# AnastasiaBelenkii/tendermint

Measured on AMD Instinct MI355X. Metric: ed25519 verifies/sec at 1/2/4/8 GPUs + p50 VerifyCommit latency, 150 vals, higher is better.
Workload: dtype int32

## Files before the change

__graft_entry__.py:

```python
import os
import subprocess
import sys

REPO = os.path.dirname(os.path.abspath(__file__))


def build() -> None:
    env = dict(os.environ, PYTORCH_ROCM_ARCH="gfx950")
    subprocess.run(["make", "-s", "-C", os.path.join(REPO, "tendermint_amd", "csrc")], check=True, env=env)
    subprocess.run(["bash", os.path.join(REPO, "tools", "build_checks.sh")], check=True, env=env)
    subprocess.run(["make", "-s", "-C", os.path.join(REPO, "oracle")], check=True)
    subprocess.run(["make", "-s", "-C", os.path.join(REPO, "tendermint_amd", "testing", "csrc")], check=True)
    subprocess.run(["make", "-s", "-C", os.path.join(REPO, "tests", "native")], check=True)
    subprocess.run(["make", "-s", "-C", os.path.join(REPO, "tests", "native", "secp")], check=True)
    subprocess.run(["make", "-s", "-C", os.path.join(REPO, "tests", "native", "secpcomb")], check=True)
    subprocess.run(["make", "-s", "-C", os.path.join(REPO, "tests", "native", "merkle")], check=True)
    subprocess.run(["make", "-s", "-C", os.path.join(REPO, "tests", "native", "pcache")], check=True)
    subprocess.run(["make", "-s", "-C", os.path.join(REPO, "tests", "native", "colorder")], check=True)
    subprocess.run(["make", "-s", "-C", os.path.join(REPO, "tests", "native", "split")], check=True)
    subprocess.run(["make", "-s", "-C", os.path.join(REPO, "tests", "native", "blocks")], check=True)
    subprocess.run(["make", "-s", "-C", os.path.join(REPO, "tests", "native", "voteext")], check=True)
    subprocess.run(["make", "-s", "-C", os.path.join(REPO, "tests", "native", "proofops")], check=True)
    subprocess.run(["make", "-s", "-C", os.path.join(REPO, "tests", "native", "stage")], check=True)
    subprocess.run(["make", "-s", "-C", os.path.join(REPO, "tests", "native", "results")], check=True)
    subprocess.run(["make", "-s", "-C", os.path.join(REPO, "tests", "native", "keyorder")], check=True)
    subprocess.run(["make", "-s", "-C", os.path.join(REPO, "tests", "native", "blockwire")], check=True)
    sys.path.insert(0, REPO)
    import tendermint_amd
    from tendermint_amd import _native
    _native.lib()


def smoke() -> None:
    sys.path.insert(0, REPO)
    sys.path.insert(0, os.path.join(REPO, "oracle"))
    import numpy as np
    import torch
    from tendermint_amd import _native
    from tendermint_amd.testing.factory import make_c2_batch
    import oracle_c

    assert torch.cuda.is_available(), "smoke() needs a GPU"
    ctx = _native.Context(1)
    b = make_c2_batch(1000, seed=7)
    ok_g, vec_g = ctx.ed25519_verify_batch(b.pk, b.sig, b.msg, b.off)
    ok_o, vec_o = oracle_c.ed25519_verify_packed(b.pk, b.sig, b.msg, b.off, threads=4)
    assert ok_g == ok_o and np.array_equal(vec_g, vec_o), "GPU validity vector differs from the oracle"
    info = _native.build_info()
    print(f"smoke ok: {int(vec_g.sum())}/{b.n} valid, bit-exact vs oracle; {info['version']} "
          f"(src digest of this tree {'matches' if info['src_match'] else 'DIFFERS: ' + info['src_digest_tree']})")


if __name__ == "__main__":
    build()
    smoke()
```

tendermint_amd/csrc/msm.h:

```cpp
#pragma once
#include <stddef.h>
#include <stdint.h>
#include "curve25519.h"
#include "split.h"

namespace tmv {

constexpr uint32_t kMsmWideRows = 65536;
constexpr int kMsmChunkMax = 32;
constexpr uint32_t kMsmEmpty = 0xffffffffu;
constexpr uint32_t kMsmCompactGroups = 2048;
constexpr uint32_t kMsmSplitGroups = 4096;
constexpr uint32_t kMsmSplitMax = 8;
constexpr int kMsmSortBlock = 256;
constexpr uint32_t kSubGroupLog2 = 3;
constexpr uint32_t kSubGroup = 1u << kSubGroupLog2;

struct alignas(16) niels_pt {
  fe ypx, ymx, xy2d;
  int32_t pad[2];
};

#ifndef TMV_NIELS_PAIR
#define TMV_NIELS_PAIR 0
#endif
constexpr uint32_t kNielsPer = TMV_NIELS_PAIR ? 2 : 1;

TMV_HD niels_pt niels_negate(const niels_pt &p) {
  niels_pt r;
  r.ypx = p.ymx;
  r.ymx = p.ypx;
  fe_neg(r.xy2d, p.xy2d);
  r.pad[0] = r.pad[1] = 0;
  return r;
}

TMV_HD void niels_store(niels_pt *pts, uint64_t i, const niels_pt &p) {
  if (kNielsPer == 2) {
    pts[2 * i] = p;
    pts[2 * i + 1] = niels_negate(p);
  } else {
    pts[i] = p;
  }
}

struct MsmParams {
  uint32_t m_log2;
  uint32_t c;
  uint32_t W;
  uint32_t WR;
  uint32_t H;
  uint32_t cap;
  uint32_t groups;
  uint32_t P;
  uint32_t L;
  uint32_t merged;
  uint32_t sub;
  uint32_t Ws;
  uint32_t Wa;
  uint32_t Wl;
  uint32_t split_max;
  uint32_t split;

  TMV_HD uint32_t m() const { return 1u << m_log2; }
  TMV_HD uint32_t WL() const { return (129 + m_log2 + c - 1) / c; }
  TMV_HD uint32_t buckets_per_group() const { return W * H; }
  TMV_HD uint32_t bucket(uint32_t w, uint32_t i) const { return w * H + i; }
  TMV_HD uint32_t chunks_per_group() const { return cap / L; }
  TMV_HD uint32_t wpart_slots() const { return P; }

  static MsmParams make(uint32_t n, uint32_t m_log2, uint32_t c, bool merged = false) {
    MsmParams p;
    p.m_log2 = m_log2;
    p.c = c;
    p.merged = merged ? 1 : 0;
    p.sub = 0;
    p.WR = (129 + c - 1) / c;
    p.W = merged ? p.WR : (254 + c - 1) / c;
    p.H = 1u << (c - 1);
    const uint32_t m = 1u << m_log2;
    const uint32_t rw = p.WR > p.WL() ? p.WR : p.WL();
    const uint32_t slots = merged ? m * p.WR : m * rw + (m + 1) * p.W;
    p.cap = (slots + kMsmChunkMax - 1) / kMsmChunkMax * kMsmChunkMax;
    const uint32_t mean = (merged ? m : 2 * m) / p.H;
    p.L = mean <= 16 ? 16 : 32;
    p.groups = (n + m - 1) >> m_log2;
    uint32_t best = ~0u;
    for (uint32_t P = 1; P <= p.H; P *= 2) {
      uint32_t lg = 0;
      while ((p.H / P) >> (lg + 1)) lg++;
      const uint32_t chain = 2 * (p.H / P) + 3 * P + lg;
      if (chain < best) { best = chain; p.P = P; }
    }
    if ((uint64_t)p.groups * p.W >= kMsmWideRows) p.P = 1;
    p.Ws = split_windows(p.W);
    p.Wa = p.Ws > p.WR ? p.Ws : p.WR;
    p.Wl = p.Ws > p.WL() ? p.Ws : p.WL();
    p.split_max = 0;
    p.split = 0;
    return p;
  }
};

struct MsmWork {
  niels_pt *pts;
  uint32_t *ent_pt;
  uint32_t *ent_bk;
  uint32_t *bk_start;
  uint32_t *bk_cnt;
  ge_p3 *bk_sum;
  ge_p3 *part_first;
  ge_p3 *part_last;
  uint32_t *join_b;
  uint32_t *join_count;
  ge_p3 *wpart;
  ge_p3 *wsum;
  uint32_t *grp_chunks;
  uint32_t *chunk_end;
  uint32_t compact;
  uint8_t *group_ok;
  uint8_t *sort_ovf;
  uint32_t n_pts;
  uint32_t *fail_count;
  uint32_t *fail_list;
  uint8_t *sub_ok;
  fe *tabR;
  fe *fail_T;
  uint32_t *loc_count;
  uint32_t *fb_count;
  uint32_t *loc_found;
  uint32_t *fb_list;
  const uint8_t *merge_pk;
  uint8_t *grp_split;
  uint32_t *hi_of;
  uint32_t *hi_list;
  uint32_t *uns_list;
  uint32_t *split_cnt;
  uint32_t g_base;
  unsigned long long *ent_total;
  uint32_t *wscal;
  uint32_t *bscal;
  fe *item_pt;

  static size_t max_items(uint32_t n, const MsmParams &p) { return (size_t)n + 2ull * p.groups; }

  static size_t point_slots(uint32_t n, const MsmParams &p) {
    return 2ull * n + 1 + (p.split ? 1 + (size_t)p.groups * p.split_max : 0);
  }
  static size_t bytes(uint32_t n, const MsmParams &p) {
    const size_t G = p.groups, bk = (size_t)G * p.buckets_per_group(), ent = (size_t)G * p.cap;
    const size_t chunks = ent / p.L;
    size_t b = point_slots(n, p) * kNielsPer * sizeof(niels_pt) + 8 * ent + 8 * bk + bk * sizeof(ge_p3) +
// ... 160 lines not shown
```

tendermint_amd/csrc/msm_kernels.hip:

```cpp
#include <hip/hip_runtime.h>
#include <cstdlib>
#include <cstring>
#include "ed25519_core.h"
#include "kernel_util.h"
#include "comb.h"
#include "quad.h"
#include "ktimer.h"
#include "verify_kernels.h"
#include "halfscalar.h"
#include "knobs.h"

#include <algorithm>
#include <atomic>
#include <mutex>
#include <vector>

namespace tmv {

namespace ktimer {
namespace {
struct Pair {
  int k;
  hipEvent_t a, b;
};
std::atomic<bool> g_on{false};
std::mutex g_mu;
std::vector<Pair *> g_done[kCount];
std::vector<hipEvent_t> g_free;
hipEvent_t take_event() {
  hipEvent_t e = nullptr;
  {
    std::lock_guard<std::mutex> lk(g_mu);
    if (!g_free.empty()) { e = g_free.back(); g_free.pop_back(); }
  }
  if (!e && hipEventCreate(&e) != hipSuccess) e = nullptr;
  return e;
}
}

void set(bool on) { g_on.store(on); }
bool on() { return g_on.load(std::memory_order_relaxed); }

void *begin(Kernel k, hipStream_t s) {
  if (!on()) return nullptr;
  Pair *p = new Pair{k, take_event(), take_event()};
  if (!p->a || !p->b || hipEventRecord(p->a, s) != hipSuccess) {
    std::lock_guard<std::mutex> lk(g_mu);
    if (p->a) g_free.push_back(p->a);
    if (p->b) g_free.push_back(p->b);
    delete p;
    return nullptr;
  }
  return p;
}

void end(void *token, hipStream_t s) {
  if (!token) return;
  Pair *p = static_cast<Pair *>(token);
  (void)hipEventRecord(p->b, s);
  std::lock_guard<std::mutex> lk(g_mu);
  g_done[p->k].push_back(p);
}

int read(Kernel k, double *ms, uint64_t *launches) {
  std::vector<Pair *> v;
  {
    std::lock_guard<std::mutex> lk(g_mu);
    v.swap(g_done[k]);
  }
  int rc = 0;
  for (Pair *p : v) {
    float t = 0.f;
    hipError_t e = hipEventSynchronize(p->b);
    if (e == hipSuccess) e = hipEventElapsedTime(&t, p->a, p->b);
    if (e == hipSuccess) {
      *ms += t;
      *launches += 1;
    } else if (!rc) {
      rc = (int)e;
    }
    std::lock_guard<std::mutex> lk(g_mu);
    g_free.push_back(p->a);
    g_free.push_back(p->b);
    delete p;
  }
  return rc;
}

}

namespace {

template <int V>
struct StaticIndex {
  static constexpr int value = V;
};

template <int NW>
struct DigitReader {
  uint32_t wd[NW];
  uint64_t buf;
  uint32_t avail;
  int carry;
  __device__ __forceinline__ void init(const uint32_t *s) {
#pragma unroll
    for (int k = 0; k < NW; k++) wd[k] = s[k];
    buf = 0;
    avail = 0;
    carry = 0;
  }
  __device__ __forceinline__ int next(uint32_t c, bool top) {
    if (avail < c) {
      buf |= (uint64_t)wd[0] << avail;
#pragma unroll
      for (int k = 0; k + 1 < NW; k++) wd[k] = wd[k + 1];
      wd[NW - 1] = 0;
      avail += 32;
    }
    int d = (int)(buf & ((1u << c) - 1)) + carry;
    buf >>= c;
    avail -= c;
    if (!top && d >= (1 << (c - 1))) {
      d -= 1 << c;
      carry = 1;
    } else {
      carry = 0;
    }
    return d;
  }
};

template <int NW, typename F>
__device__ __forceinline__ void for_each_digit(const uint32_t *s, uint32_t windows, const MsmParams &p, F f) {
  DigitReader<NW> rd;
  rd.init(s);
  for (uint32_t w = 0; w < windows; w++) {
    const int d = rd.next(p.c, w + 1 == windows);
    if (d != 0) f(p.bucket(w, (uint32_t)((d < 0 ? -d : d) - 1)), d < 0);
  }
}

__device__ __forceinline__ void p3_add(ge_p3 &a, const ge_p3 &b) {
  ge_cached c;
  ge_p3_to_cached(c, b);
  ge_p1p1 r;
  ge_add(r, a, c);
  ge_p1p1_to_p3(a, r);
}

TMV_HD uint32_t merge_runs(const MsmParams &p) { return p.m() / 2 < 256u ? p.m() / 2 : 256u; }

constexpr uint32_t kSplitWords = 40;
TMV_HD uint32_t sort_words(const MsmParams &p, uint32_t bs) {
  const uint32_t sort = bs * 9 + bs + 1 + 2 * (2 * p.m() + 1);
  const uint32_t merge = 6 * p.m() + 1 + 16 * merge_runs(p);
  return p.W * p.H + (sort > merge ? sort : merge);
}

__device__ __forceinline__ void p3_dbl(ge_p3 &a) {
  ge_p1p1 r;
  ge_p3_dbl(r, a);
  ge_p1p1_to_p3(a, r);
}

}

template <bool SR, bool KM, int BS = kMsmSortBlock, bool LOC = false, bool SPLIT = false>
__global__ void __launch_bounds__(BS)
k_msm_sort(const uint8_t *__restrict__ sig, const uint32_t *__restrict__ idx, const uint32_t *count_ptr, uint32_t n,
           Ed25519Work w, MsmWork mw, MsmParams p, MsmSeed seed, const fe *__restrict__ btab_q, int aligned,
           const uint32_t *__restrict__ key_slot, const uint8_t *__restrict__ key_ok, uint8_t *__restrict__ out,
           uint32_t e_base) {
  extern __shared__ uint32_t smem[];
  const uint32_t cnt = entry_count(count_ptr, n);
  const uint32_t tid = threadIdx.x;
  uint32_t g = blockIdx.x;
  if (g == 0 && tid == 0) *mw.join_count = 0;
  if (LOC) {
    const uint32_t nf = *mw.fail_count;
    if (g == 0 && tid == 0) {
      *mw.loc_count = nf << p.m_log2;
      *mw.fb_count = 0;
      *mw.loc_found = 0;
    }
    if (g >= nf) return;
  }
  const uint32_t slot = g;
  if (LOC) g = mw.fail_list[slot];
  const uint32_t e0 = g << p.m_log2;
  if (!KM && !LOC && g == 0 && tid == 0) {
    niels_pt bp;
    bp.ymx = btab_q[0];
    bp.ypx = btab_q[1];
    bp.xy2d = btab_q[2];
    bp.pad[0] = bp.pad[1] = 0;
    niels_store(mw.pts, mw.n_pts, bp);
    if constexpr (SPLIT) {
      const fe *bh = btab_q + 4 * (2 * kBaseQuadEntries + (p.c - 4));
      bp.ymx = bh[0];
      bp.ypx = bh[1];
      bp.xy2d = bh[2];
      niels_store(mw.pts, mw.n_pts + 1, bp);
    }
    if (mw.fail_count) *mw.fail_count = 0;
  }
  if (e0 >= cnt) return;
  const uint32_t mlive = min(p.m(), cnt - e0);
  const uint32_t WH = p.W * p.H;
  uint32_t *hist = smem;
  uint32_t *red = smem + WH;
  uint32_t *scan = red + BS * 9;

  constexpr int R = 4;
  constexpr int ZW = LOC ? 5 : 4;
  const uint32_t WRz = LOC ? p.WL() : p.WR;
  uint32_t z[R][ZW], wv[R][8];
  bool live[R];
  uint32_t acc[9];
#pragma unroll
  for (int t = 0; t < 9; t++) acc[t] = 0;
  auto weigh = [&](auto rc) {
// ... 165 lines not shown
        if (diff) continue;
        follower[r] = true;
        trun[myslot[r]] = kWant;
      }
      __syncthreads();
#pragma unroll
      for (int r = 0; r < R; r++) {
        if (!leader[r] || trun[myslot[r]] != kWant) continue;
        const uint32_t sl = atomicAdd(nruns, 1u);
        trun[myslot[r]] = sl < RUNS ? sl : kNone;
      }
      __syncthreads();
#pragma unroll
      for (int r = 0; r < R; r++) {
        if (!follower[r]) continue;
        const uint32_t sl = trun[myslot[r]];
        if (sl >= RUNS) continue;
#pragma unroll
        for (int t = 0; t < 8; t++) {
          atomicAdd(&racc[sl * 16 + 2 * t], wv[r][t] & 0xffffu);
          atomicAdd(&racc[sl * 16 + 2 * t + 1], wv[r][t] >> 16);
          wv[r][t] = 0;
        }
      }
      __syncthreads();
#pragma unroll
      for (int r = 0; r < R; r++) {
        if (!leader[r]) continue;
        const uint32_t sl = trun[myslot[r]];
        if (sl >= RUNS) continue;
        uint32_t x[16];
        uint64_t c = 0;
#pragma unroll
        for (int t = 0; t < 8; t++) {
          c += (uint64_t)racc[sl * 16 + 2 * t] + (wv[r][t] & 0xffffu);
          const uint32_t lo16 = (uint32_t)c & 0xffffu;
          c >>= 16;
          c += (uint64_t)racc[sl * 16 + 2 * t + 1] + (wv[r][t] >> 16);
          x[t] = lo16 | (((uint32_t)c & 0xffffu) << 16);
          c >>= 16;
        }
        x[8] = (uint32_t)c;
#pragma unroll
        for (int t = 9; t < 16; t++) x[t] = 0;
        sc_reduce512(wv[r], x);
      }
    }
  }

  bool split_g = false;
  uint32_t hi_pt[R];
  int carry_hi[R], carry_bhi = 0;
  uint32_t *lmask = smem + sort_words(p, BS), *lbad = lmask + 32, *lbase = lmask + 33;
  if constexpr (SPLIT) {
    bool lead[R];
#pragma unroll
    for (int r = 0; r < R; r++) {
      hi_pt[r] = 0;
      carry_hi[r] = 0;
      uint32_t nz = 0;
#pragma unroll
      for (int t = 0; t < 8; t++) nz |= wv[r][t];
      lead[r] = live[r] && nz != 0;
    }
    if (tid < 34) lmask[tid] = 0;
    __syncthreads();
#pragma unroll
    for (int r = 0; r < R; r++) {
      const uint32_t j = tid + r * BS;
      if (lead[r]) atomicOr(&lmask[j >> 5], 1u << (j & 31));
    }
    __syncthreads();
    uint32_t leaders = 0;
    for (uint32_t k = 0; k < (p.m() + 31) / 32; k++) leaders += __popc(lmask[k]);
    split_g = LOC ? mw.grp_split[g] != 0 : leaders <= p.split_max;
    if (tid == 0) {
      mw.grp_split[(LOC ? p.groups : 0) + slot] = split_g ? 1 : 0;
      if (!split_g) {
        mw.uns_list[atomicAdd(&mw.split_cnt[1], 1u)] = slot;
      } else if (!LOC) {
        *lbase = atomicAdd(&mw.split_cnt[0], leaders);
        if (mw.ent_total) {
          atomicAdd(&mw.ent_total[4], 1ull);
          atomicAdd(&mw.ent_total[5], (unsigned long long)leaders);
        }
      }
    }
    if (split_g) {
      if (!LOC) __syncthreads();
#pragma unroll
      for (int r = 0; r < R; r++) {
        if (!live[r]) continue;
        const uint32_t j = tid + r * BS, e = e0 + j;
        uint32_t gslot = kMsmEmpty;
        if (LOC) {
          if (lead[r]) {
            gslot = mw.hi_of[e];
            if (gslot == kMsmEmpty) atomicOr(lbad, 1u);
          }
        } else {
          if (lead[r]) {
            uint32_t rank = __popc(lmask[j >> 5] & ((1u << (j & 31)) - 1));
            for (uint32_t k = 0; k < (j >> 5); k++) rank += __popc(lmask[k]);
            gslot = (mw.g_base + g) * p.split_max + rank;
            mw.hi_list[2 * (*lbase + rank)] = e;
            mw.hi_list[2 * (*lbase + rank) + 1] = gslot;
          }
          mw.hi_of[e] = gslot;
        }
        hi_pt[r] = mw.n_pts + 2 + gslot;
      }
    }
  }
  auto count_split = [&](const uint32_t *s, int &cy) {
    DigitReader<8> rd;
    rd.init(s);
    for (uint32_t w = 0; w < p.W; w++) {
      if (w == p.Ws) cy = rd.carry;
      const int d = rd.next(p.c, w + 1 == p.W);
      if (d != 0) atomicAdd(&hist[p.bucket(split_slot(w, p.Ws, split_g).window, (uint32_t)((d < 0 ? -d : d) - 1))], 1u);
    }
  };

#pragma unroll
  for (int r = 0; r < R; r++) {
    if (!live[r]) continue;
    for_each_digit<ZW>(z[r], WRz, p, [&](uint32_t bk, bool) { atomicAdd(&hist[bk], 1u); });
    if constexpr (SPLIT) count_split(wv[r], carry_hi[r]);
    else if (!KM) for_each_digit<8>(wv[r], p.W, p, [&](uint32_t bk, bool) { atomicAdd(&hist[bk], 1u); });
  }
  if constexpr (SPLIT) {
    if (tid == 0) count_split(bsc, carry_bhi);
  } else {
    if (!KM && tid == 0) for_each_digit<8>(bsc, p.W, p, [&](uint32_t bk, bool) { atomicAdd(&hist[bk], 1u); });
  }
  __syncthreads();

  const uint32_t seg = (WH + BS - 1) / BS;
  const uint32_t lo = min(WH, tid * seg), hi = min(WH, lo + seg);
  uint32_t local = 0;
  for (uint32_t t = lo; t < hi; t++) local += hist[t];
  scan[tid] = local;
  __syncthreads();
  if (tid == 0) {
    uint32_t run = 0;
    for (int t = 0; t < BS; t++) {
      const uint32_t v = scan[t];
      scan[t] = run;
      run += v;
    }
    scan[BS] = run;
  }
  __syncthreads();
  const uint32_t gbase = slot * p.cap;
  const uint32_t bbase = slot * WH;
  const bool ovf = scan[BS] > p.cap || (SPLIT && *lbad != 0);
  if (tid == 0) mw.sort_ovf[(LOC ? p.groups : 0) + slot] = ovf ? 1 : 0;
  if (tid == 0 && !ovf && mw.ent_total) atomicAdd(mw.ent_total, (unsigned long long)scan[BS]);
  if (tid == 0) mw.grp_chunks[slot] = ovf ? 0u : (scan[BS] + p.L - 1) / p.L;
  if (ovf) {
    for (uint32_t t = tid; t < WH; t += BS) {
      mw.bk_start[bbase + t] = gbase;
      mw.bk_cnt[bbase + t] = 0;
    }
    for (uint32_t t = tid; t < p.cap; t += BS) mw.ent_bk[gbase + t] = kMsmEmpty;
    return;
  }
  {
    uint32_t off = scan[tid];
    for (uint32_t t = lo; t < hi; t++) {
      const uint32_t c = hist[t];
      mw.bk_start[bbase + t] = gbase + off;
      mw.bk_cnt[bbase + t] = c;
      hist[t] = off;
      off += c;
    }
  }
  __syncthreads();

  uint32_t *ent_pt = mw.ent_pt + gbase;
  uint32_t *ent_bk = mw.ent_bk + gbase;
  const uint32_t wcap = 2 * p.m() + 1;
  uint32_t *st_pt = scan + BS + 1, *st_bk = st_pt + wcap;
  DigitReader<ZW> rz[R];
  const uint32_t total = scan[BS];
  if constexpr (SPLIT) {
    DigitReader<5> rlo[R], rblo;
    DigitReader<4> rhi[R], rbhi;
    const uint32_t sh = p.c * p.Ws;
    auto high_half = [&](DigitReader<4> &rd, const uint32_t *s, int cy) {
      uint32_t t[9], h[4];
#pragma unroll
      for (int k = 0; k < 8; k++) t[k] = s[k];
      t[8] = 0;
      for (uint32_t i = 0; i < (sh >> 5); i++) {
#pragma unroll
        for (int k = 0; k < 8; k++) t[k] = t[k + 1];
      }
#pragma unroll
      for (int k = 0; k < 4; k++) h[k] = (uint32_t)((((uint64_t)t[k + 1] << 32) | t[k]) >> (sh & 31));
      rd.init(h);
      rd.carry = cy;
    };
#pragma unroll
    for (int r = 0; r < R; r++) {
      rz[r].init(z[r]);
      rlo[r].init(wv[r]);
      high_half(rhi[r], wv[r], carry_hi[r]);
    }
    rblo.init(bsc);
    high_half(rbhi, bsc, carry_bhi);
    const uint32_t Wg = split_g ? (LOC ? p.Wl : p.Wa) : p.W;
    for (uint32_t w = 0; w < Wg; w++) {
      const uint32_t wbeg = hist[p.bucket(w, 0)];
      const uint32_t wend = w + 1 < p.W ? hist[p.bucket(w + 1, 0)] : total;
      __syncthreads();
      auto put = [&](int d, uint32_t pt) {
        if (d == 0) return;
        const uint32_t bk = p.bucket(w, (uint32_t)((d < 0 ? -d : d) - 1));
        const uint32_t pos = atomicAdd(&hist[bk], 1u) - wbeg;
        st_pt[pos] = (pt << 1) | (d < 0 ? 1u : 0u);
        st_bk[pos] = bbase + bk;
      };
      const uint32_t wh = split_g ? w + p.Ws : w;
      const bool lo_on = w < p.Ws, hi_on = wh >= p.Ws && wh < p.W;
#pragma unroll
      for (int r = 0; r < R; r++) {
        if (!live[r]) continue;
        const uint32_t e = e0 + tid + r * BS;
        if (w < WRz) put(rz[r].next(p.c, w + 1 == WRz), 2 * e);
        if (lo_on) put(rlo[r].next(p.c, false), 2 * e + 1);
        if (hi_on) put(rhi[r].next(p.c, wh + 1 == p.W), split_g ? hi_pt[r] : 2 * e + 1);
      }
      if (tid == 0) {
        if (lo_on) put(rblo.next(p.c, false), mw.n_pts);
        if (hi_on) put(rbhi.next(p.c, wh + 1 == p.W), split_g ? mw.n_pts + 1 : mw.n_pts);
      }
      __syncthreads();
      for (uint32_t i = tid; i < wend - wbeg; i += BS) {
        ent_pt[wbeg + i] = st_pt[i];
        ent_bk[wbeg + i] = st_bk[i];
      }
    }
    const uint32_t pad_end = mw.compact ? min(p.cap, (total + p.L - 1) / p.L * p.L) : p.cap;
    for (uint32_t t = total + tid; t < pad_end; t += BS) ent_bk[t] = kMsmEmpty;
    return;
  }
  DigitReader<8> rw[R], rb;
#pragma unroll
  for (int r = 0; r < R; r++) {
    rz[r].init(z[r]);
    rw[r].init(wv[r]);
  }
  rb.init(bsc);
  for (uint32_t w = 0; w < p.W; w++) {
    const uint32_t wbeg = hist[p.bucket(w, 0)];
    const uint32_t wend = w + 1 < p.W ? hist[p.bucket(w + 1, 0)] : total;
    __syncthreads();
#pragma unroll
    for (int r = 0; r < R; r++) {
      if (!live[r]) continue;
      const uint32_t e = e0 + tid + r * BS;
      if (w < WRz) {
        const int d = rz[r].next(p.c, w + 1 == WRz);
        if (d != 0) {
          const uint32_t bk = p.bucket(w, (uint32_t)((d < 0 ? -d : d) - 1));
          const uint32_t pos = atomicAdd(&hist[bk], 1u) - wbeg;
          st_pt[pos] = ((KM ? e : 2 * e) << 1) | (d < 0 ? 1u : 0u);
          st_bk[pos] = bbase + bk;
        }
      }
      if (!KM) {
        const int d = rw[r].next(p.c, w + 1 == p.W);
        if (d != 0) {
          const uint32_t bk = p.bucket(w, (uint32_t)((d < 0 ? -d : d) - 1));
          const uint32_t pos = atomicAdd(&hist[bk], 1u) - wbeg;
          st_pt[pos] = ((2 * e + 1) << 1) | (d < 0 ? 1u : 0u);
          st_bk[pos] = bbase + bk;
        }
      }
    }
    if (!KM && tid == 0) {
      const int d = rb.next(p.c, w + 1 == p.W);
      if (d != 0) {
        const uint32_t bk = p.bucket(w, (uint32_t)((d < 0 ? -d : d) - 1));
        const uint32_t pos = atomicAdd(&hist[bk], 1u) - wbeg;
        st_pt[pos] = (mw.n_pts << 1) | (d < 0 ? 1u : 0u);
        st_bk[pos] = bbase + bk;
      }
    }
    __syncthreads();
    for (uint32_t i = tid; i < wend - wbeg; i += BS) {
      ent_pt[wbeg + i] = st_pt[i];
      ent_bk[wbeg + i] = st_bk[i];
    }
  }
  const uint32_t pad_end = mw.compact ? min(p.cap, (total + p.L - 1) / p.L * p.L) : p.cap;
  for (uint32_t t = total + tid; t < pad_end; t += BS) ent_bk[t] = kMsmEmpty;
// ... 791 lines not shown

static Ed25519Work work_view(Ed25519Work w, uint64_t e0) {
  w.negA += 4 * e0;
  w.Rc += 4 * e0;
  w.k += 8 * e0;
  w.flags += 4 * e0;
  w.tabA += 64 * e0;
  w.hs_buf += 12 * e0;
  w.miss_list += e0;
  w.miss_count += e0 >> 5;
  return w;
}
static MsmWork msm_view(MsmWork mw, const MsmParams &p, uint32_t n, uint64_t g0) {
  const uint64_t e0 = g0 << p.m_log2, wh = (uint64_t)p.W * p.H;
  mw.pts += 2 * e0 * kNielsPer;
  mw.n_pts = (uint32_t)(2ull * n - 2 * e0);
  mw.ent_pt += g0 * p.cap;
  mw.ent_bk += g0 * p.cap;
  mw.bk_start += g0 * wh;
  mw.bk_cnt += g0 * wh;
  mw.bk_sum += g0 * wh;
  mw.part_first += g0 * p.chunks_per_group();
  mw.part_last += g0 * p.chunks_per_group();
  mw.join_b += g0 * p.chunks_per_group();
  mw.join_count += g0;
  mw.grp_chunks += g0;
  mw.chunk_end += g0;
  mw.wpart += g0 * p.W * 2ull * p.P;
  mw.wsum += g0 * p.W;
  mw.group_ok += g0;
  mw.sort_ovf += g0;
  if (mw.grp_split) {
    mw.grp_split += g0;
    mw.hi_of += e0;
    mw.hi_list += 2 * g0 * p.split_max;
    mw.uns_list += g0;
    mw.split_cnt += 2 * g0;
    mw.g_base = (uint32_t)g0;
  }
  if (mw.sub_ok) mw.sub_ok += (g0 << p.m_log2) / kSubGroup;
  if (mw.tabR) mw.tabR += 32 * e0;
  return mw;
}

template <bool SR, bool LOC>
static hipError_t launch_sort(const uint8_t *sig, const uint32_t *idx, const uint32_t *count_ptr, uint32_t n,
                              uint32_t e_base, const fe *btab_q, Ed25519Work w, MsmWork mw, const MsmParams &p,
                              const MsmSeed &seed, uint8_t *out, int aligned, hipStream_t stream) {
  mw.compact = compact_on(p) ? 1 : 0;
  if constexpr (!SR) {
    if (split_on(mw, p)) {
      hipError_t e = hipMemsetAsync(mw.split_cnt, 0, 2 * sizeof(uint32_t), stream);
      if (e != hipSuccess) return e;
      if (p.m_log2 <= 8)
        hipLaunchKernelGGL((k_msm_sort<false, false, 64, LOC, true>), dim3(p.groups), dim3(64), sort_smem(p, 64, true),
                           stream, sig, idx, count_ptr, n, w, mw, p, seed, btab_q, aligned, nullptr, nullptr, out,
                           e_base);
      else
        hipLaunchKernelGGL((k_msm_sort<false, false, kMsmSortBlock, LOC, true>), dim3(p.groups), dim3(kMsmSortBlock),
                           sort_smem(p, kMsmSortBlock, true), stream, sig, idx, count_ptr, n, w, mw, p, seed, btab_q,
                           aligned, nullptr, nullptr, out, e_base);
      return hipGetLastError();
    }
  }
  if (p.m_log2 <= 8)
    hipLaunchKernelGGL((k_msm_sort<SR, false, 64, LOC>), dim3(p.groups), dim3(64), sort_smem(p, 64), stream, sig, idx,
                       count_ptr, n, w, mw, p, seed, btab_q, aligned, nullptr, nullptr, out, e_base);
  else
    hipLaunchKernelGGL((k_msm_sort<SR, false, kMsmSortBlock, LOC>), dim3(p.groups), dim3(kMsmSortBlock),
                       sort_smem(p, kMsmSortBlock), stream, sig, idx, count_ptr, n, w, mw, p, seed, btab_q, aligned,
                       nullptr, nullptr, out, e_base);
  return hipGetLastError();
}

template <bool SR>
static hipError_t launch_part(const uint8_t *pk, const uint8_t *sig, const uint8_t *msg, const uint32_t *msg_off,
                              const uint32_t *idx, const uint32_t *count_ptr, uint32_t n, uint32_t e_base,
                              const fe *btab_q, const strobe_t *prefix, Ed25519Work w, MsmWork mw,
                              const MsmParams &p, const MsmSeed &seed, uint8_t *out, int aligned,
                              hipStream_t stream) {
  w.niels = mw.pts;
  hipError_t e = launch_prep<SR>(pk, sig, msg, msg_off, idx, count_ptr, n, prefix, w, aligned, stream);
  if (e != hipSuccess) return e;
  if ((e = launch_sort<SR, false>(sig, idx, count_ptr, n, e_base, btab_q, w, mw, p, seed, out, aligned, stream)) !=
      hipSuccess)
    return e;
  if (split_on(mw, p)) {
    const uint64_t hb = ((uint64_t)p.groups * p.split_max + kHiBlock / 4 - 1) / (kHiBlock / 4);
    hipLaunchKernelGGL(k_msm_hi_points, dim3((uint32_t)hb), dim3(kHiBlock), 0, stream, w, mw, p);
    if ((e = hipGetLastError()) != hipSuccess) return e;
  }
  return launch_buckets(count_ptr, n, mw, p, stream);
}

template <bool SR>
static hipError_t launch_tail_stages(const uint8_t *sig, const uint32_t *idx, const uint32_t *count_ptr, uint32_t n,
                                     const fe *btab_q, Ed25519Work w, MsmWork mw, const MsmParams &p,
                                     const MsmSeed &seed, uint8_t *out, int aligned, hipStream_t stream) {
  hipError_t e;
  const bool located = locate_enabled(n, p);
  const bool split = split_on(mw, p);
  const uint8_t *gsplit = split ? mw.grp_split : nullptr;
  const bool helped = !located && w.hs_buf && !split;
  const uint32_t hblocks = (p.groups + 15) / 16;
  if (helped) {
    hipLaunchKernelGGL(k_msm_horner_helped<SR>, dim3(hblocks + (n + 63) / 64), dim3(64), 0, stream, count_ptr, n, mw,
                       p, w, hblocks);
// ... 260 lines not shown
```

tendermint_amd/csrc/tmverify_runtime.cpp:

```cpp
#include <hip/hip_runtime.h>
#include <sys/random.h>

#include <cerrno>

#include <algorithm>
#include <array>
#include <atomic>
#include <chrono>
#include <cstdint>
#include <list>
#include <unordered_map>
#include <cstdlib>
#include <cstdio>
#include <cstring>
#include <functional>
#include <memory>
#include <condition_variable>
#include <mutex>
#include <string>
#include <thread>
#include <vector>

#include "../../include/tmverify.h"
#include "ed25519_core.h"
// ... 359 lines not shown
    if (e == hipErrorNotReady) return 1;
    err = e;
    return 2;
  }, g_timeout_ms);
  if (r == tmh::Poll::kTimeout) {
    d.faulted = true;
    set_error("device wait exceeded TMV_DEVICE_TIMEOUT_MS (" + std::to_string(g_timeout_ms) + " ms)");
    return hipErrorNotReady;
  }
  return err;
}
hipError_t wait_event(Device &d, hipEvent_t ev) {
  read_env();
  hipError_t err = hipSuccess;
  const tmh::Poll r = tmh::poll_until([&] {
    const hipError_t e = hipEventQuery(ev);
    if (e == hipSuccess) return 0;
    if (e == hipErrorNotReady) return 1;
    err = e;
    return 2;
  }, g_timeout_ms);
  if (r == tmh::Poll::kTimeout) {
    d.faulted = true;
    set_error("device wait exceeded TMV_DEVICE_TIMEOUT_MS (" + std::to_string(g_timeout_ms) + " ms)");
    return hipErrorNotReady;
  }
  return err;
}
int wait_rc(hipError_t e) { return e == hipErrorNotReady ? TMV_ERR_TIMEOUT : TMV_ERR_LAUNCH; }
int faulted_rc(Device &d) {
  set_error("device timed out earlier (TMV_ERR_TIMEOUT); open a new context");
  return TMV_ERR_TIMEOUT;
}
int use_device(Device &d, void *stream = nullptr, hipStream_t *s = nullptr) {
  const hipError_t e = hipSetDevice(d.id);
  if (e != hipSuccess) { set_error("hipSetDevice", e); return TMV_ERR_NO_DEVICE; }
  if (!s) return 0;
  *s = stream ? static_cast<hipStream_t>(stream) : context_stream(d);
  if (!*s) { set_error("hipStreamCreate failed"); return TMV_ERR_NO_DEVICE; }
  return 0;
}

constexpr double kRunningSumWeight = 3.0;
static double running_sum_weight() {
  const char *e = tmv::ab_knob("TMV_RS_WEIGHT");
  return e ? atof(e) : kRunningSumWeight;
}
static std::atomic<uint32_t> g_split_groups{tmv::kMsmSplitGroups};
static std::atomic<uint32_t> g_split_max{tmv::kMsmSplitMax};
static uint32_t split_max() {
  const char *e = tmv::ab_knob("TMV_SPLIT_MAX");
  return e ? (uint32_t)strtoul(e, nullptr, 10) : g_split_max.load(std::memory_order_relaxed);
}
tmv::MsmParams msm_params(uint32_t n, uint32_t m_log2, uint32_t c, bool merged = false, bool ed_only = false,
                          int sub = -1) {
  const uint32_t lmin = tmv::locate_min_entries();
  if (m_log2 == 0) m_log2 = merged ? 8 : (ed_only && lmin && n >= lmin ? 7 : 6);
  m_log2 = std::max<uint32_t>(5, std::min<uint32_t>(10, m_log2));
  if (c == 0) {
    const double m = double(1u << m_log2), rsw = running_sum_weight();
    double best = 1e30;
    for (uint32_t cc = 4; cc <= 9; cc++) {
      const double W = (254 + cc - 1) / cc, WR = (129 + cc - 1) / cc, H = double(1u << (cc - 1));
      const double cost = merged ? m * WR + 2.2 * WR * H : m * (W + WR) + rsw * W * H;
      if (cost < best) { best = cost; c = cc; }
    }
  }
  c = std::max<uint32_t>(4, std::min<uint32_t>(9, c));
  tmv::MsmParams p = tmv::MsmParams::make(n, m_log2, c, merged);
  if (g_msm_chunk == 16 || g_msm_chunk == 32) p.L = g_msm_chunk;
  if (g_msm_parts && g_msm_parts <= p.H && !(g_msm_parts & (g_msm_parts - 1))) p.P = g_msm_parts;
  p.sub = merged ? 0 : (sub < 0 ? (tmv::subcheck_enabled(m_log2) ? 1 : 0) : (uint32_t)sub);
  const uint32_t sg = g_split_groups.load(std::memory_order_relaxed);
  const uint32_t smax = tmv::split_max_for(p.m(), split_max());
  if (!merged && ed_only && smax && (sg == 1 || (p.P == 1 && p.groups >= sg)) &&
      2ull * n + 2 + (uint64_t)p.groups * smax < (1ull << 31)) {
    p.split = 1;
    p.split_max = smax;
    p.P = 1;
  }
  return p;
}

struct EngineTimer {
  bool on = tmh::host_timing();
  std::chrono::steady_clock::time_point t = std::chrono::steady_clock::now();
  void mark(const char *what, uint32_t n) {
    if (!on) return;
    const auto now = std::chrono::steady_clock::now();
    fprintf(stderr, "[tmv_engine] %-8s %9.3f ms (n=%u)\n", what,
            std::chrono::duration<double, std::milli>(now - t).count(), n);
    t = now;
  }
};

struct Layout {
  size_t pk, sig, off, msg, total;
  Layout(uint32_t n, size_t msg_bytes) {
    pk = 0;
    sig = align16(pk + 32ull * n);
    off = align16(sig + 64ull * n);
    msg = align16(off + 4ull * (n + 1));
    total = align16(msg + std::max<size_t>(msg_bytes, 1));
  }
};

struct LaunchOpts {
  bool batch_eq = false;
  tmv::MsmParams p{};
  tmv::MsmParams p_ed{};
  tmv::MsmParams p_ed_streamed{};
  tmv::MsmSeed seed[2]{};
  int err = 0;
  bool stats = false;
};

std::atomic<int> g_rand_fault_err{0}, g_rand_fault_count{0};

int draw_weight_key(uint8_t key[32]) {
  size_t got = 0;
  while (got < 32) {
    ssize_t r;
    int fc = g_rand_fault_count.load();
    if (fc != 0) {
      if (fc > 0) g_rand_fault_count.fetch_sub(1);
      errno = g_rand_fault_err.load();
      r = -1;
    } else {
      r = getrandom(key + got, 32 - got, 0);
    }
    if (r > 0) {
// ... 818 lines not shown
  else if (!strcmp(kernel, "k_merkle_aunts")) k = tmv::ktimer::kMerkleAunts;
  else if (!strcmp(kernel, "k_merkle_verify_proofs")) k = tmv::ktimer::kMerkleVerify;
  else if (!strcmp(kernel, "k_merkle_leaves")) k = tmv::ktimer::kMerkleLeaves;
  else if (!strcmp(kernel, "k_commit_leaves")) k = tmv::ktimer::kCommitLeaves;
  else if (!strcmp(kernel, "k_vote_ext_signbytes")) k = tmv::ktimer::kVoteExtSignbytes;
  else if (!strcmp(kernel, "k_merkle_digests_long")) k = tmv::ktimer::kMerkleDigestsLong;
  else if (!strcmp(kernel, "k_merkle_value_ops")) k = tmv::ktimer::kMerkleValueOps;
  else if (!strcmp(kernel, "k_result_leaves")) k = tmv::ktimer::kResultLeaves;
  else if (!strcmp(kernel, "k_span_leaves")) k = tmv::ktimer::kSpanLeaves;
  else { set_error("unknown timed kernel"); return TMV_ERR_ARG; }
  *total_ms = 0;
  *launches = 0;
  const int e = tmv::ktimer::read(k, total_ms, launches);
  if (e) { set_error("hipEventElapsedTime", (hipError_t)e); return TMV_ERR_LAUNCH; }
  return 0;
}

const char *tmv_last_error(void) { return g_last_error.c_str(); }
void tmv_internal_set_error(const char *msg) { g_last_error = msg ? msg : ""; }

void tmv_internal_random_fault(int err, int count) {
  g_rand_fault_err = err;
  g_rand_fault_count = count;
}
int tmv_internal_option(const char *name, int64_t value) {
  if (name && !strcmp(name, "half_scalars")) {
    tmv::set_half_scalar_mode((int)value);
    return 0;
  }
  if (name && !strcmp(name, "point_cache_min")) {
    tmv::set_point_cache_min(value < 0 ? 0u : (uint32_t)value);
    return 0;
  }
  if (name && !strcmp(name, "column_tile")) {
    g_column_tile = value;
    return 0;
  }
  if (name && !strcmp(name, "compact_groups")) {
    tmv::set_compact_groups(value < 0 ? 0u : (uint32_t)value);
    return 0;
  }
  if (name && !strcmp(name, "key_merge")) {
    tmv::set_key_merge(value != 0);
    return 0;
  }
  if (name && !strcmp(name, "split_groups")) {
    g_split_groups = value <= 0 ? tmv::kMsmSplitGroups : (uint32_t)value;
    return 0;
  }
  if (name && !strcmp(name, "split_max")) {
    g_split_max = value <= 0 ? tmv::kMsmSplitMax : (uint32_t)value;
    return 0;
  }
  set_error("unknown internal option");
  return TMV_ERR_ARG;
}
int tmv_internal_checks(uint32_t *out3, int reset) {
  if (!out3) { set_error("null argument"); return TMV_ERR_ARG; }
  if (!tmv::read_checks(out3, reset != 0)) {
    set_error("not a TMV_CHECKS build, or the device read failed");
    return TMV_ERR_ARG;
  }
  return 0;
}
int64_t tmv_internal_mixed_stream_chunk(uint64_t free_bytes) {
  read_env();
  return mixed_stream_chunk((size_t)free_bytes);
}
int tmv_internal_draw_key(uint8_t *out32) {
  if (!out32) { set_error("null argument"); return TMV_ERR_ARG; }
  return draw_weight_key(out32);
}

tmv_ctx *tmv_open(uint32_t device_mask) { return tmv_open_logical(device_mask, 1); }

tmv_ctx *tmv_open_logical(uint32_t device_mask, int logical) {
  release_leaked_pins();
  int count = 0;
  hipError_t e = hipGetDeviceCount(&count);
  if (e != hipSuccess || count <= 0) {
    set_error(e != hipSuccess ? std::string("hipGetDeviceCount: ") + hipGetErrorString(e)
                              : std::string("no HIP device visible"));
    return nullptr;
  }
  logical = std::max(1, std::min(8, logical));
  if (logical > 1)
    fprintf(stderr, "tmverify: TEST AID tmv_open_logical: every GPU opened as %d logical devices\n", logical);
  auto ctx = std::make_unique<tmv_ctx>();
  for (int i = 0; i < count && i < 32; i++) {
    if (device_mask != 0 && !(device_mask & (1u << i))) continue;
    for (int k = 0; k < logical; k++) {
      auto d = std::make_unique<Device>();
      d->id = i;
      if (init_device(*d) != 0) {
        tmv_close(ctx.release());
        return nullptr;
      }
      ctx->devs.push_back(std::move(d));
    }
  }
  if (ctx->devs.empty()) {
    set_error("device_mask selects no visible device");
    return nullptr;
  }
  return ctx.release();
}
// ... 1253 lines not shown
```

Measured before the change: 245.7 million.

## Spread split-scalar leader digit work across thread lanes in MSM sort

In the split path of the MSM sort kernel, each leader scalar's low and high halves (plus the base scalar) become separate tasks, each handled by its own thread. The tasks are staged through a shared-memory table so histogram and scatter run in parallel instead of serially per leader and on thread 0 for the base scalar. This is meant to shorten the serial tail of the sort kernel. In exchange it adds shared-memory staging, a launch-bounds occupancy hint for the split variant, and a cap on split_max tied to the sort block size.

Measured after the change: 245.6 million, median of 4. No clear change (-0.0%).

```diff
diff --git a/__graft_entry__.py b/__graft_entry__.py
--- a/__graft_entry__.py
+++ b/__graft_entry__.py
@@ -18,6 +18,7 @@
     subprocess.run(["make", "-s", "-C", os.path.join(REPO, "tests", "native", "pcache")], check=True)
     subprocess.run(["make", "-s", "-C", os.path.join(REPO, "tests", "native", "colorder")], check=True)
     subprocess.run(["make", "-s", "-C", os.path.join(REPO, "tests", "native", "split")], check=True)
+    subprocess.run(["make", "-s", "-C", os.path.join(REPO, "tests", "native", "splitlanes")], check=True)
     subprocess.run(["make", "-s", "-C", os.path.join(REPO, "tests", "native", "blocks")], check=True)
     subprocess.run(["make", "-s", "-C", os.path.join(REPO, "tests", "native", "voteext")], check=True)
     subprocess.run(["make", "-s", "-C", os.path.join(REPO, "tests", "native", "proofops")], check=True)
diff --git a/tendermint_amd/csrc/msm.h b/tendermint_amd/csrc/msm.h
--- a/tendermint_amd/csrc/msm.h
+++ b/tendermint_amd/csrc/msm.h
@@ -3,6 +3,7 @@
 #include <stdint.h>
 #include "curve25519.h"
 #include "split.h"
+#include "split_lanes.h"
 
 namespace tmv {
 
@@ -13,6 +14,7 @@
 constexpr uint32_t kMsmSplitGroups = 4096;
 constexpr uint32_t kMsmSplitMax = 8;
 constexpr int kMsmSortBlock = 256;
+TMV_HD uint32_t sort_block(uint32_t m_log2) { return m_log2 <= 8 ? 64u : (uint32_t)kMsmSortBlock; }
 constexpr uint32_t kSubGroupLog2 = 3;
 constexpr uint32_t kSubGroup = 1u << kSubGroupLog2;
 
@@ -61,6 +63,7 @@
   uint32_t Wl;
   uint32_t split_max;
   uint32_t split;
+  uint32_t lanes;
 
   TMV_HD uint32_t m() const { return 1u << m_log2; }
   TMV_HD uint32_t WL() const { return (129 + m_log2 + c - 1) / c; }
@@ -98,6 +101,7 @@
     p.Wl = p.Ws > p.WL() ? p.Ws : p.WL();
     p.split_max = 0;
     p.split = 0;
+    p.lanes = 0;
     return p;
   }
 };
diff --git a/tendermint_amd/csrc/msm_kernels.hip b/tendermint_amd/csrc/msm_kernels.hip
--- a/tendermint_amd/csrc/msm_kernels.hip
+++ b/tendermint_amd/csrc/msm_kernels.hip
@@ -9,6 +9,7 @@
 #include "verify_kernels.h"
 #include "halfscalar.h"
 #include "knobs.h"
+#include "split_lanes.h"
 
 #include <algorithm>
 #include <atomic>
@@ -96,40 +97,6 @@
   static constexpr int value = V;
 };
 
-template <int NW>
-struct DigitReader {
-  uint32_t wd[NW];
-  uint64_t buf;
-  uint32_t avail;
-  int carry;
-  __device__ __forceinline__ void init(const uint32_t *s) {
-#pragma unroll
-    for (int k = 0; k < NW; k++) wd[k] = s[k];
-    buf = 0;
-    avail = 0;
-    carry = 0;
-  }
-  __device__ __forceinline__ int next(uint32_t c, bool top) {
-    if (avail < c) {
-      buf |= (uint64_t)wd[0] << avail;
-#pragma unroll
-      for (int k = 0; k + 1 < NW; k++) wd[k] = wd[k + 1];
-      wd[NW - 1] = 0;
-      avail += 32;
-    }
-    int d = (int)(buf & ((1u << c) - 1)) + carry;
-    buf >>= c;
-    avail -= c;
-    if (!top && d >= (1 << (c - 1))) {
-      d -= 1 << c;
-      carry = 1;
-    } else {
-      carry = 0;
-    }
-    return d;
-  }
-};
-
 template <int NW, typename F>
 __device__ __forceinline__ void for_each_digit(const uint32_t *s, uint32_t windows, const MsmParams &p, F f) {
   DigitReader<NW> rd;
@@ -166,7 +133,7 @@
 }
 
 template <bool SR, bool KM, int BS = kMsmSortBlock, bool LOC = false, bool SPLIT = false>
-__global__ void __launch_bounds__(BS)
+__global__ void __launch_bounds__(BS, SPLIT ? 3 : 1)
 k_msm_sort(const uint8_t *__restrict__ sig, const uint32_t *__restrict__ idx, const uint32_t *count_ptr, uint32_t n,
            Ed25519Work w, MsmWork mw, MsmParams p, MsmSeed seed, const fe *__restrict__ btab_q, int aligned,
            const uint32_t *__restrict__ key_slot, const uint8_t *__restrict__ key_ok, uint8_t *__restrict__ out,
@@ -438,6 +405,28 @@
   uint32_t hi_pt[R];
   int carry_hi[R], carry_bhi = 0;
   uint32_t *lmask = smem + sort_words(p, BS), *lbad = lmask + 32, *lbase = lmask + 33;
+  constexpr uint32_t kLaneWords = 10;
+  static_assert((BS / 2) * kLaneWords <= BS * 9, "the task table fits red");
+  bool lanes_g = false;
+  uint32_t ntask = 0;
+  auto task_reader = [&](DigitReader<5> &rd) {
+    const SplitTask task = split_task(tid);
+    const uint32_t *row = red + task.rank * kLaneWords;
+    uint32_t th[5];
+#pragma unroll
+    for (int k = 0; k < 5; k++)
+      th[k] = split_half_word([&](uint32_t q) { return row[q]; }, (uint32_t)k, task.hi, p.c, p.Ws);
+    rd.init(th);
+    if (task.hi) {
+      uint32_t s8[8];
+#pragma unroll
+      for (int t = 0; t < 8; t++) s8[t] = row[t];
+      rd.carry = split_carry_in(s8, p.c, p.Ws);
+    }
+    return row[8 + task.hi];
+  };
+  const bool ttop = (tid & 1) != 0;
+  const uint32_t tnw = ttop ? p.W - p.Ws : p.Ws;
   if constexpr (SPLIT) {
     bool lead[R];
 #pragma unroll
@@ -460,6 +449,7 @@
     uint32_t leaders = 0;
     for (uint32_t k = 0; k < (p.m() + 31) / 32; k++) leaders += __popc(lmask[k]);
     split_g = LOC ? mw.grp_split[g] != 0 : leaders <= p.split_max;
+    lanes_g = split_g && p.lanes && split_task_count(leaders) <= (uint32_t)BS;
     if (tid == 0) {
       mw.grp_split[(LOC ? p.groups : 0) + slot] = split_g ? 1 : 0;
       if (!split_g) {
@@ -478,7 +468,11 @@
       for (int r = 0; r < R; r++) {
         if (!live[r]) continue;
         const uint32_t j = tid + r * BS, e = e0 + j;
-        uint32_t gslot = kMsmEmpty;
+        uint32_t gslot = kMsmEmpty, rank = 0;
+        if (lead[r]) {
+          rank = __popc(lmask[j >> 5] & ((1u << (j & 31)) - 1));
+          for (uint32_t k = 0; k < (j >> 5); k++) rank += __popc(lmask[k]);
+        }
         if (LOC) {
           if (lead[r]) {
             gslot = mw.hi_of[e];
@@ -486,8 +480,6 @@
           }
         } else {
           if (lead[r]) {
-            uint32_t rank = __popc(lmask[j >> 5] & ((1u << (j & 31)) - 1));
-            for (uint32_t k = 0; k < (j >> 5); k++) rank += __popc(lmask[k]);
             gslot = (mw.g_base + g) * p.split_max + rank;
             mw.hi_list[2 * (*lbase + rank)] = e;
             mw.hi_list[2 * (*lbase + rank) + 1] = gslot;
@@ -495,7 +487,25 @@
           mw.hi_of[e] = gslot;
         }
         hi_pt[r] = mw.n_pts + 2 + gslot;
-      }
+        if (lanes_g && lead[r]) {
+          uint32_t *row = red + rank * kLaneWords;
+#pragma unroll
+          for (int t = 0; t < 8; t++) row[t] = wv[r][t];
+          row[8] = 2 * e + 1;
+          row[9] = hi_pt[r];
+        }
+      }
+    }
+    if (lanes_g) {
+      if (tid == 0) {
+        uint32_t *row = red + leaders * kLaneWords;
+#pragma unroll
+        for (int t = 0; t < 8; t++) row[t] = bsc[t];
+        row[8] = mw.n_pts;
+        row[9] = mw.n_pts + 1;
+      }
+      __syncthreads();
+      ntask = split_task_count(leaders);
     }
   }
   auto count_split = [&](const uint32_t *s, int &cy) {
@@ -512,11 +522,23 @@
   for (int r = 0; r < R; r++) {
     if (!live[r]) continue;
     for_each_digit<ZW>(z[r], WRz, p, [&](uint32_t bk, bool) { atomicAdd(&hist[bk], 1u); });
-    if constexpr (SPLIT) count_split(wv[r], carry_hi[r]);
-    else if (!KM) for_each_digit<8>(wv[r], p.W, p, [&](uint32_t bk, bool) { atomicAdd(&hist[bk], 1u); });
+    if constexpr (SPLIT) {
+      if (!lanes_g) count_split(wv[r], carry_hi[r]);
+    } else if (!KM) for_each_digit<8>(wv[r], p.W, p, [&](uint32_t bk, bool) { atomicAdd(&hist[bk], 1u); });
   }
   if constexpr (SPLIT) {
-    if (tid == 0) count_split(bsc, carry_bhi);
+    if (lanes_g) {
+      if (tid < ntask) {
+        DigitReader<5> rd;
+        task_reader(rd);
+        for (uint32_t w = 0; w < tnw; w++) {
+          const int d = rd.next(p.c, ttop && w + 1 == tnw);
+          if (d != 0) atomicAdd(&hist[p.bucket(w, (uint32_t)((d < 0 ? -d : d) - 1))], 1u);
+        }
+      }
+    } else if (tid == 0) {
+      count_split(bsc, carry_bhi);
+    }
   } else {
     if (!KM && tid == 0) for_each_digit<8>(bsc, p.W, p, [&](uint32_t bk, bool) { atomicAdd(&hist[bk], 1u); });
   }
@@ -571,6 +593,45 @@
   DigitReader<ZW> rz[R];
   const uint32_t total = scan[BS];
   if constexpr (SPLIT) {
+    auto scatter_windows = [&](uint32_t Wg, auto body) {
+      for (uint32_t w = 0; w < Wg; w++) {
+        const uint32_t wbeg = hist[p.bucket(w, 0)];
+        const uint32_t wend = w + 1 < p.W ? hist[p.bucket(w + 1, 0)] : total;
+        __syncthreads();
+        auto put = [&](int d, uint32_t pt) {
+          if (d == 0) return;
+          const uint32_t bk = p.bucket(w, (uint32_t)((d < 0 ? -d : d) - 1));
+          const uint32_t pos = atomicAdd(&hist[bk], 1u) - wbeg;
+          st_pt[pos] = (pt << 1) | (d < 0 ? 1u : 0u);
+          st_bk[pos] = bbase + bk;
+        };
+        body(w, put);
+        __syncthreads();
+        for (uint32_t i = tid; i < wend - wbeg; i += BS) {
+          ent_pt[wbeg + i] = st_pt[i];
+          ent_bk[wbeg + i] = st_bk[i];
+        }
+      }
+      const uint32_t pad_end = mw.compact ? min(p.cap, (total + p.L - 1) / p.L * p.L) : p.cap;
+      for (uint32_t t = total + tid; t < pad_end; t += BS) ent_bk[t] = kMsmEmpty;
+    };
+    if (lanes_g) {
+#pragma unroll
+      for (int r = 0; r < R; r++) rz[r].init(z[r]);
+      DigitReader<5> tr;
+      uint32_t tpt = 0;
+      if (tid < ntask) tpt = task_reader(tr);
+      else tr.init(z[0]);
+      scatter_windows(LOC ? p.Wl : p.Wa, [&](uint32_t w, auto put) {
+#pragma unroll
+        for (int r = 0; r < R; r++) {
+          if (!live[r]) continue;
+          if (w < WRz) put(rz[r].next(p.c, w + 1 == WRz), 2 * (e0 + tid + r * BS));
+        }
+        if (tid < ntask && w < tnw) put(tr.next(p.c, ttop && w + 1 == tnw), tpt);
+      });
+      return;
+    }
     DigitReader<5> rlo[R], rblo;
     DigitReader<4> rhi[R], rbhi;
     const uint32_t sh = p.c * p.Ws;
@@ -596,18 +657,7 @@
     }
     rblo.init(bsc);
     high_half(rbhi, bsc, carry_bhi);
-    const uint32_t Wg = split_g ? (LOC ? p.Wl : p.Wa) : p.W;
-    for (uint32_t w = 0; w < Wg; w++) {
-      const uint32_t wbeg = hist[p.bucket(w, 0)];
-      const uint32_t wend = w + 1 < p.W ? hist[p.bucket(w + 1, 0)] : total;
-      __syncthreads();
-      auto put = [&](int d, uint32_t pt) {
-        if (d == 0) return;
-        const uint32_t bk = p.bucket(w, (uint32_t)((d < 0 ? -d : d) - 1));
-        const uint32_t pos = atomicAdd(&hist[bk], 1u) - wbeg;
-        st_pt[pos] = (pt << 1) | (d < 0 ? 1u : 0u);
-        st_bk[pos] = bbase + bk;
-      };
+    scatter_windows(split_g ? (LOC ? p.Wl : p.Wa) : p.W, [&](uint32_t w, auto put) {
       const uint32_t wh = split_g ? w + p.Ws : w;
       const bool lo_on = w < p.Ws, hi_on = wh >= p.Ws && wh < p.W;
 #pragma unroll
@@ -622,14 +672,7 @@
         if (lo_on) put(rblo.next(p.c, false), mw.n_pts);
         if (hi_on) put(rbhi.next(p.c, wh + 1 == p.W), split_g ? mw.n_pts + 1 : mw.n_pts);
       }
-      __syncthreads();
-      for (uint32_t i = tid; i < wend - wbeg; i += BS) {
-        ent_pt[wbeg + i] = st_pt[i];
-        ent_bk[wbeg + i] = st_bk[i];
-      }
-    }
-    const uint32_t pad_end = mw.compact ? min(p.cap, (total + p.L - 1) / p.L * p.L) : p.cap;
-    for (uint32_t t = total + tid; t < pad_end; t += BS) ent_bk[t] = kMsmEmpty;
+    });
     return;
   }
   DigitReader<8> rw[R], rb;
@@ -1527,7 +1570,7 @@
     if (split_on(mw, p)) {
       hipError_t e = hipMemsetAsync(mw.split_cnt, 0, 2 * sizeof(uint32_t), stream);
       if (e != hipSuccess) return e;
-      if (p.m_log2 <= 8)
+      if (sort_block(p.m_log2) == 64)
         hipLaunchKernelGGL((k_msm_sort<false, false, 64, LOC, true>), dim3(p.groups), dim3(64), sort_smem(p, 64, true),
                            stream, sig, idx, count_ptr, n, w, mw, p, seed, btab_q, aligned, nullptr, nullptr, out,
                            e_base);
diff --git a/tendermint_amd/csrc/split_lanes.h b/tendermint_amd/csrc/split_lanes.h
--- /dev/null
+++ b/tendermint_amd/csrc/split_lanes.h
@@ -0,0 +1,94 @@
+#pragma once
+#include <stdint.h>
+#include "curve25519.h"
+
+namespace tmv {
+
+template <int NW>
+struct DigitReader {
+  uint32_t wd[NW];
+  uint64_t buf;
+  uint32_t avail;
+  int carry;
+  TMV_HD void init(const uint32_t *s) {
+#pragma unroll
+    for (int k = 0; k < NW; k++) wd[k] = s[k];
+    buf = 0;
+    avail = 0;
+    carry = 0;
+  }
+  TMV_HD int next(uint32_t c, bool top) {
+    if (avail < c) {
+      buf |= (uint64_t)wd[0] << avail;
+#pragma unroll
+      for (int k = 0; k + 1 < NW; k++) wd[k] = wd[k + 1];
+      wd[NW - 1] = 0;
+      avail += 32;
+    }
+    int d = (int)(buf & ((1u << c) - 1)) + carry;
+    buf >>= c;
+    avail -= c;
+    if (!top && d >= (1 << (c - 1))) {
+      d -= 1 << c;
+      carry = 1;
+    } else {
+      carry = 0;
+    }
+    return d;
+  }
+};
+
+struct SplitTask {
+  uint32_t rank;
+  uint32_t hi;
+};
+TMV_HD uint32_t split_task_count(uint32_t leaders) { return 2 * (leaders + 1); }
+TMV_HD SplitTask split_task(uint32_t t) {
+  SplitTask k;
+  k.rank = t >> 1;
+  k.hi = t & 1;
+  return k;
+}
+
+TMV_HD uint32_t split_max_lanes(uint32_t bs, uint32_t want) {
+  const uint32_t most = bs / 2 - 1;
+  return want < most ? want : most;
+}
+
+TMV_HD int split_carry_in(const uint32_t s[8], uint32_t c, uint32_t Ws) {
+  const uint32_t sh = c * Ws;
+  uint64_t cy = 0;
+  uint32_t kbit = c - 1, ki = 0;
+  int out = 0;
+  bool done = sh == 0;
+#pragma unroll
+  for (int k = 0; k < 8; k++) {
+    if (done) continue;
+    uint32_t kw = 0;
+    while (ki < Ws && kbit < 32u * (k + 1)) {
+      kw |= 1u << (kbit & 31);
+      kbit += c;
+      ki++;
+    }
+    const uint32_t rem = sh - 32u * k;
+    uint32_t sw = s[k];
+    if (rem < 32) sw &= (1u << rem) - 1;
+    cy += (uint64_t)sw + kw;
+    if (rem <= 32) {
+      out = (int)((cy >> rem) & 1);
+      done = true;
+    }
+    cy >>= 32;
+  }
+  return out;
+}
+
+template <typename F>
+TMV_HD uint32_t split_half_word(F at, uint32_t k, uint32_t hi, uint32_t c, uint32_t Ws) {
+  const uint32_t sh = hi ? c * Ws : 0;
+  const uint32_t q = (sh >> 5) + k;
+  const uint32_t a = q < 8 ? at(q) : 0, b = q + 1 < 8 ? at(q + 1) : 0;
+  return (uint32_t)((((uint64_t)b << 32) | a) >> (sh & 31));
+}
+
+}
diff --git a/tendermint_amd/csrc/tmverify_runtime.cpp b/tendermint_amd/csrc/tmverify_runtime.cpp
--- a/tendermint_amd/csrc/tmverify_runtime.cpp
+++ b/tendermint_amd/csrc/tmverify_runtime.cpp
@@ -435,6 +435,11 @@
   const char *e = tmv::ab_knob("TMV_SPLIT_MAX");
   return e ? (uint32_t)strtoul(e, nullptr, 10) : g_split_max.load(std::memory_order_relaxed);
 }
+static std::atomic<uint32_t> g_leader_lanes{1};
+static uint32_t leader_lanes() {
+  const char *e = tmv::ab_knob("TMV_LEADER_LANES");
+  return e ? (uint32_t)strtoul(e, nullptr, 10) : g_leader_lanes.load(std::memory_order_relaxed);
+}
 tmv::MsmParams msm_params(uint32_t n, uint32_t m_log2, uint32_t c, bool merged = false, bool ed_only = false,
                           int sub = -1) {
   const uint32_t lmin = tmv::locate_min_entries();
@@ -455,11 +460,13 @@
   if (g_msm_parts && g_msm_parts <= p.H && !(g_msm_parts & (g_msm_parts - 1))) p.P = g_msm_parts;
   p.sub = merged ? 0 : (sub < 0 ? (tmv::subcheck_enabled(m_log2) ? 1 : 0) : (uint32_t)sub);
   const uint32_t sg = g_split_groups.load(std::memory_order_relaxed);
-  const uint32_t smax = tmv::split_max_for(p.m(), split_max());
+  const uint32_t smax =
+      tmv::split_max_lanes(tmv::sort_block(p.m_log2), tmv::split_max_for(p.m(), split_max()));
   if (!merged && ed_only && smax && (sg == 1 || (p.P == 1 && p.groups >= sg)) &&
       2ull * n + 2 + (uint64_t)p.groups * smax < (1ull << 31)) {
     p.split = 1;
     p.split_max = smax;
+    p.lanes = leader_lanes() ? 1 : 0;
     p.P = 1;
   }
   return p;
@@ -1384,6 +1391,10 @@
     g_split_max = value <= 0 ? tmv::kMsmSplitMax : (uint32_t)value;
     return 0;
   }
+  if (name && !strcmp(name, "leader_lanes")) {
+    g_leader_lanes = value < 0 ? 1u : (value ? 1u : 0u);
+    return 0;
+  }
   set_error("unknown internal option");
   return TMV_ERR_ARG;
 }
```
